# JorisAR/GDPathTracing

Measured on AMD Instinct MI355X. Metric: Mrays/sec at 1920x1080, 8 spp, 4 bounces, higher is better.
Workload: dtype f32

## Files before the change

### gdpathtracing_amd/csrc/jpt_kernels_wf2.hip

```cpp
#include <algorithm>
#include <cstdlib>

#include "jpt_trace_core.h"
#include "jpt_tie_walk.h"
#include "jpt_tuning.h"
#include "jpt_variance.h"

#ifndef JPT_PRIMARY_WAVES
#define JPT_PRIMARY_WAVES 7
#endif

namespace jpt {

namespace {

constexpr int kBlock = kTraceBlock;
constexpr uint32_t kSegments = 256u * JPT_WAVES_PER_SIMD;
struct WfTune {
    int refill_idle;
    int primary_refill_idle;
    int node_min_lanes;
    int leaf_min_lanes;
    int inst_min_lanes;
    int phase_frac16;
    int tail_rounds;
    int tail_lanes;
};

template <bool COUNT, bool W4>
__device__ __forceinline__ bool walk_round(Traversal<COUNT, W4>& tr, bool active, const WideSceneDev& sc,
                                           const typename Traversal<COUNT, W4>::Stack& st, DevCounters& cnt, const WfTune& tune, uint32_t& steps)
{
    const int kNodeMinLanes = tune.node_min_lanes;
    const bool lane0 = (threadIdx.x & 63) == 0;
    if (COUNT && lane0) cnt.phase[0]++;
    const int na = __popcll(__ballot(active));
    const int cap = (na * tune.phase_frac16) >> 4;
    const int lmin = tune.leaf_min_lanes < cap ? tune.leaf_min_lanes : cap;
    const int imin = tune.inst_min_lanes < cap ? tune.inst_min_lanes : cap;
    for (int it = 0; it < 64; it++) {
        if (active && !tr.have && tr.sp > 0) tr.pop_next(st);
        const bool want = active && tr.wants_node();
        const unsigned long long m = __ballot(want);
        if (m == 0 || (it > 0 && __popcll(m) < kNodeMinLanes)) break;
        if (COUNT && lane0) {
            cnt.phase[1]++;
            cnt.phase[2] += (unsigned long long)__popcll(m);
        }
        if (want) tr.node_step(sc, st, cnt);
        if (COUNT && want) steps++;
    }
    bool wl = active && tr.wants_leaf();
    bool wi = active && tr.wants_instance();
    if (W4 && (tune.leaf_min_lanes > 1 || tune.inst_min_lanes > 1)) {
        const int nl = __popcll(__ballot(wl)), ni = __popcll(__ballot(wi));
        const bool nodes_left = __any(active && tr.wants_node()) || __any(active && !tr.have && tr.sp > 0);
        const bool run_l = nl >= lmin || !(nodes_left || ni >= imin);
        const bool run_i = ni >= imin || !(nodes_left || (run_l && nl > 0));
        wl = wl && run_l;
        wi = wi && run_i;
    }
    if (COUNT) {
        const int nl = __popcll(__ballot(wl)), ni = __popcll(__ballot(wi));
        if (lane0 && nl) {
            cnt.phase[3]++;
            cnt.phase[4] += (unsigned long long)nl;
        }
        if (lane0 && ni) {
            cnt.phase[5]++;
            cnt.phase[6] += (unsigned long long)ni;
        }
    }
    if (wl) tr.leaf_step(sc, cnt);
    if (wi) tr.instance_step(sc, st, cnt);
    if (COUNT && (wl || wi)) steps++;
    return active && tr.finished();
}

__device__ __forceinline__ bool in_mask(const unsigned long long m) { return __builtin_amdgcn_inverse_ballot_w64(m); }

struct WalkMasks {
    unsigned long long have = 0ull, in_blas = 0ull;
};
template <bool COUNT, bool W4>
__device__ __forceinline__ unsigned long long walk_round_masked(Traversal<COUNT, W4>& tr, typename Traversal<COUNT, W4>::Masked& ml, WalkMasks& wm,
                                                                const unsigned long long act, const WideSceneDev& sc,
                                                                const typename Traversal<COUNT, W4>::Stack& st, DevCounters& cnt, const WfTune& tune,
                                                                uint32_t& steps)
{
    using Walk = Traversal<COUNT, W4>;
    const int kNodeMinLanes = tune.node_min_lanes;
    const bool lane0 = (threadIdx.x & 63) == 0;
    if (COUNT && lane0) cnt.phase[0]++;
    const int na = __popcll(act);
    const int cap = (na * tune.phase_frac16) >> 4;
    const int lmin = tune.leaf_min_lanes < cap ? tune.leaf_min_lanes : cap;
    const int imin = tune.inst_min_lanes < cap ? tune.inst_min_lanes : cap;
    const uint32_t base = Walk::lds_base(st);
    unsigned long long have_m = wm.have, blas_m = wm.in_blas;
    for (int it = 0; it < 64; it++) {
        const unsigned long long pm = act & ~have_m & __ballot(ml.top > base);
        if (pm) {
            if (in_mask(pm)) tr.cur = tr.pop_at(st, ml.top);
            const unsigned long long sent = pm & __ballot(tr.cur == kSentinel);
            have_m |= pm & ~sent;
            if (sent) {
                blas_m &= ~sent;
                const unsigned long long more = sent & __ballot(ml.top > base);
                if (in_mask(more)) {
                    tr.cur = tr.pop_at(st, ml.top);
                    if (!Walk::kLean || tr.cur >= 0) tr.restore_world();
                }
                have_m |= more;
            }
        }
        const unsigned long long m = act & have_m & __ballot(tr.cur >= 0);
        if (m == 0 || (it > 0 && __popcll(m) < kNodeMinLanes)) break;
        if (COUNT && lane0) {
            cnt.phase[1]++;
            cnt.phase[2] += (unsigned long long)__popcll(m);
        }
        const bool want = in_mask(m);
        ml.in_blas = in_mask(blas_m);
        if (want) tr.template node_step<true>(sc, st, cnt, &ml);
        if (COUNT && want) steps++;
        have_m = (have_m & ~m) | (m & __ballot(ml.k0 < Walk::kNoChild));
    }
    const unsigned long long lf = __ballot(tr.cur < 0), sm = __ballot(ml.top > base);
    const unsigned long long hv = act & have_m;
    unsigned long long wlm = hv & lf & blas_m, wim = hv & lf & ~blas_m;
    if (W4 && (tune.leaf_min_lanes > 1 || tune.inst_min_lanes > 1)) {
        const int nl = __popcll(wlm), ni = __popcll(wim);
        const bool nodes_left = ((hv & ~lf) | (act & ~have_m & sm)) != 0ull;
        const bool run_l = nl >= lmin || !(nodes_left || ni >= imin);
        const bool run_i = ni >= imin || !(nodes_left || (run_l && nl > 0));
        wlm = run_l ? wlm : 0ull;
        wim = run_i ? wim : 0ull;
    }
    if (COUNT) {
        const int nl = __popcll(wlm), ni = __popcll(wim);
        if (lane0 && nl) {
            cnt.phase[3]++;
            cnt.phase[4] += (unsigned long long)nl;
        }
        if (lane0 && ni) {
            cnt.phase[5]++;
            cnt.phase[6] += (unsigned long long)ni;
        }
    }
    const bool wl = in_mask(wlm), wi = in_mask(wim);
    if (wl) tr.leaf_step(sc, cnt);
    if (wi) tr.template instance_step<true>(sc, st, cnt, &ml);
    if (COUNT && (wl || wi)) steps++;
    have_m = (have_m & ~wlm) | wim;
    blas_m |= wim;
    wm.have = have_m;
    wm.in_blas = blas_m;
    return act & ~have_m & ~sm;
}

typedef float jpt_v4f __attribute__((ext_vector_type(4)));
typedef uint32_t jpt_v4u __attribute__((ext_vector_type(4)));
__device__ __forceinline__ float4 stream_ld4(const float4* p)
{
    const jpt_v4f v = __builtin_nontemporal_load(reinterpret_cast<const jpt_v4f*>(p));
    return make_float4(v.x, v.y, v.z, v.w);
}
__device__ __forceinline__ void stream_st4(float4* p, const float4 v)
{
    jpt_v4f w;
    w.x = v.x; w.y = v.y; w.z = v.z; w.w = v.w;
    __builtin_nontemporal_store(w, reinterpret_cast<jpt_v4f*>(p));
}
__device__ __forceinline__ uint4 stream_ldu4(const uint4* p)
{
    const jpt_v4u v = __builtin_nontemporal_load(reinterpret_cast<const jpt_v4u*>(p));
    return make_uint4(v.x, v.y, v.z, v.w);
}
__device__ __forceinline__ void stream_stf(float* p, const float v) { __builtin_nontemporal_store(v, p); }
__device__ __forceinline__ uint32_t stream_ldu(const uint32_t* p) { return __builtin_nontemporal_load(p); }
__device__ __forceinline__ void stream_stu(uint32_t* p, const uint32_t v) { __builtin_nontemporal_store(v, p); }

constexpr uint32_t kHasRadiance = 0x80000000u;
constexpr uint32_t kPathMask = 0x7fffffffu;

struct Wf2Buffers {
    float4* ray_o[2];
    float4* ray_d[2];
    float4* hit_a;
    uint32_t* hit_b;
    float4* thr_q[2];
    float4* thr;
    float4* rad;
    uint32_t* fin8;
    float* first_depth;
    uint32_t* qcount;
    uint32_t* redo_count;
    float4* redo_rec;
    uint32_t redo_cap;
};

struct FastDiv {
    uint32_t d, m;
};
inline FastDiv make_fastdiv(uint32_t d) { return FastDiv{d ? d : 1u, d > 1u ? (uint32_t)(0x100000000ull / d) : 0xffffffffu}; }
__device__ __forceinline__ uint32_t fdiv(uint32_t n, const FastDiv& f)
{
    uint32_t q = __umulhi(n, f.m);
    const uint32_t r = n - q * f.d;
    return r >= f.d ? q + 1u : q;
}

struct Wf2Dims {
    int32_t tile_x0, tile_y0;
    int32_t tiles_x, tiles_y;
    int32_t full_tiles_x, full_tiles_y;
    uint32_t tiles_per_frame;
    uint32_t slots_per_frame;
    uint32_t n_chunks;
    uint32_t seg_cap;
    uint32_t run_shift;
    FastDiv by_tiles_x, by_full_tiles_x;
    FastDiv by_frames;
    int32_t acc_groups = 1;
};

__device__ __forceinline__ void slot_to_pixel(uint32_t slot, const Wf2Dims& dm, int& px, int& ly)
{
    const uint32_t tile = slot >> 6, lane = slot & 63u;
    const uint32_t ty = fdiv(tile, dm.by_tiles_x), tx = tile - ty * (uint32_t)dm.tiles_x;
    const uint32_t ix = lane & 7u, iy = lane >> 3;
    px = (int)((tx + (uint32_t)dm.tile_x0) * 8u + ix);
    ly = (int)((ty + (uint32_t)dm.tile_y0) * 8u + iy);
}

__device__ __forceinline__ void path_slot_frame(uint32_t path, const Wf2Dims& dm, uint32_t n_frames, uint32_t& slot, uint32_t& f)
{
    slot = fdiv(path, dm.by_frames);
    f = path - slot * n_frames;
}

__device__ __forceinline__ void store_final(const Wf2Buffers& wb, int accum_mode, uint32_t p, f3 r)
{
    if (accum_mode == 0) stream_stu(&wb.fin8[p], unorm8(r.x) | (unorm8(r.y) << 8) | (unorm8(r.z) << 16));
    else stream_st4(&wb.rad[p], make_float4(r.x, r.y, r.z, 0.0f));
}

__device__ __forceinline__ bool sky_culled(const SkyCull& cull, int px, int py)
{
    bool outside = cull.n >= 0;
    for (int k = 0; k < 4; k++)
        if (k < cull.n && px >= cull.x0[k] && px <= cull.x1[k] && py >= cull.y0[k] && py <= cull.y1[k]) outside = false;
    return outside;
}

__device__ __forceinline__ uint32_t lanes_below(unsigned long long mask, int lane)
{
    return (uint32_t)__popcll(mask & ((1ull << lane) - 1ull));
}

constexpr int kCoopPool = 64;

__device__ __forceinline__ float wave_min_f(float v)
{
    for (int off = 32; off > 0; off >>= 1) v = fmin_(v, __shfl_xor(v, off));
    return v;
}

template <bool COUNT>
__device__ __forceinline__ TraceHit coop_walk(const WideSceneDev& sc, const typename Traversal<COUNT, true>::Stack st, int32_t* __restrict__ pool,
                                           f3 ro, f3 rd, DevCounters& cnt, const uint32_t pool_stride = 64u)
{
    using Walk = Traversal<COUNT, true>;
    const int lane = threadIdx.x & 63;
    auto pw = [&](uint32_t w) -> int32_t& { return pool[(w >> 6) * pool_stride + (w & 63u)]; };
    constexpr uint32_t kNone = 0xffffffffu;
    Walk tr;
    tr.begin(sc, ro, rd);
    tr.hit.tri = kNone;
    bool active = lane == 0 && tr.have;
    if (lane != 0) tr.have = false;
    uint32_t n_pool = 0;
    uint32_t my_steps = 0;
    for (;;) {
        {
            const unsigned long long idle = __ballot(!active);
            const uint32_t n_idle = (uint32_t)__popcll(idle);
            const uint32_t take = n_pool < n_idle ? n_pool : n_idle;
            if (take) {
                const uint32_t r = lanes_below(idle, lane);
                if (!active && r < take) {
                    const int32_t ref = pw(2u * (n_pool - 1u - r));
                    const uint32_t ctx = (uint32_t)pw(2u * (n_pool - 1u - r) + 1u);
                    tr.sp = 0;
                    tr.cur = ref;
                    tr.have = true;
                    tr.in_blas = (ctx & 1u) != 0u;
                    tr.cur_inst = ctx >> 1;
                    if (tr.in_blas) {
                        const WideInstance* ip = sc.instances + tr.cur_inst;
                        const float4 m0 = ld4(&ip->inv[0]), m1 = ld4(&ip->inv[4]), m2 = ld4(&ip->inv[8]);
                        tr.o = mk3(m0.x * ro.x + m0.w * ro.y + m1.z * ro.z + m2.y, m0.y * ro.x + m1.x * ro.y + m1.w * ro.z + m2.z,
                                   m0.z * ro.x + m1.y * ro.y + m2.x * ro.z + m2.w);
                        tr.d = mk3(m0.x * rd.x + m0.w * rd.y + m1.z * rd.z, m0.y * rd.x + m1.x * rd.y + m1.w * rd.z,
                                   m0.z * rd.x + m1.y * rd.y + m2.x * rd.z);
                    } else {
                        tr.o = ro;
                        tr.d = rd;
                    }
                    tr.set_level();
                    active = true;
                }
                n_pool -= take;
            }
        }
        if (!__any(active)) break;
        if (COUNT && active && (tr.have || tr.sp > 0)) my_steps++;
        if (active && !tr.step(sc, st, cnt)) active = false;
        {
            const float t = wave_min_f(tr.hit.t);
            if (t < tr.hit.t) {
                tr.hit.t = t;
                tr.hit.tri = kNone;
                tr.hit.inst = 0u;
            }
        }
        {
            const uint32_t n_idle = (uint32_t)__popcll(__ballot(!active));
            const uint32_t want = n_idle > n_pool ? n_idle - n_pool : 0u;
            if (want) {
                int32_t top = kSentinel;
                const bool may = active && tr.sp > 0;
                if (may) {
                    const int row = tr.sp - 1;
                    top = row < st.lds_entries ? st.lds[row * st.stride] : (row < st.lds_entries + st.spill_entries ? st.spill[row - st.lds_entries] : kSentinel);
                }
                const bool give = may && top != kSentinel;
                const unsigned long long gm = __ballot(give);
                const uint32_t r = lanes_below(gm, lane);
                const uint32_t room = (uint32_t)kCoopPool - n_pool;
                const uint32_t lim = want < room ? want : room;
                if (give && r < lim) {
                    tr.sp--;
                    pw(2u * (n_pool + r)) = top;
                    pw(2u * (n_pool + r) + 1u) = (int32_t)((tr.in_blas ? 1u : 0u) | (tr.cur_inst << 1));
                }
                const uint32_t given = (uint32_t)__popcll(gm);
                n_pool += given < lim ? given : lim;
            }
        }
        __builtin_amdgcn_fence(__ATOMIC_RELEASE, "wavefront");
        __builtin_amdgcn_wave_barrier();
    }
    if (COUNT) {
        for (int off = 32; off > 0; off >>= 1) my_steps += (uint32_t)__shfl_xor((int)my_steps, off);
        if (lane == 0) count_walk(cnt, my_steps);
    }
    const float best = wave_min_f(tr.hit.t);
    const unsigned long long win = __ballot(tr.hit.tri != kNone && tr.hit.t == best);
    TraceHit out;
    out.t = 1e9f;
    out.u = out.v = 0.0f;
    out.tri = out.inst = 0u;
    out.front = false;
    if (win && best < 1e9f) {
        unsigned long long pick = win;
        if (__popcll(win) > 1) {
            const bool mine = ((win >> lane) & 1ull) != 0ull;
            uint32_t kt = mine ? tr.hit.tri : 0u;
            for (int off = 32; off > 0; off >>= 1) {
                const uint32_t o = (uint32_t)__shfl_xor((int)kt, off);
                kt = o > kt ? o : kt;
            }
            const bool top = mine && tr.hit.tri == kt;
            uint32_t ki = top ? ((tr.hit.inst >> kInstBits) & kInstMask) : 0u;
            for (int off = 32; off > 0; off >>= 1) {
                const uint32_t o = (uint32_t)__shfl_xor((int)ki, off);
                ki = o > ki ? o : ki;
            }
            pick = __ballot(top && ((tr.hit.inst >> kInstBits) & kInstMask) == ki);
        }
        const int w = __ffsll((long long)pick) - 1;
        out.t = best;
        out.u = __shfl(tr.hit.u, w);
        out.v = __shfl(tr.hit.v, w);
        out.tri = (uint32_t)__shfl((int)tr.hit.tri, w);
        out.front = __shfl((int)tr.hit.front, w) != 0;
        const uint32_t wi = (uint32_t)__shfl((int)tr.hit.inst, w);
        const uint32_t found_in = (wi >> kInstBits) & kInstMask;
        const bool tied = __popcll(win) > 1 || (wi & kHitTied) != 0u;
        out.inst = found_in | (found_in << kInstBits) | (tied ? kHitTied : 0u);
    }
    return out;
}

template <bool COUNT>
__device__ __attribute__((noinline)) void coop_walk_call(const WideSceneDev* __restrict__ scp, int32_t* lds_col, int32_t* pool, float ox, float oy,
                                                         float oz, float dx, float dy, float dz, DevCounters* cntp, TraceHit* out)
{
    int32_t spill[kStackSpill + 2];
    const typename Traversal<COUNT, true>::Stack st{lds_col, spill, kTraceBlock, kStackLds - 2, kStackSpill + 2};
    const WideSceneDev sc = *scp;
    DevCounters none = {};
    *out = coop_walk<COUNT>(sc, st, pool, mk3(ox, oy, oz), mk3(dx, dy, dz), COUNT ? *cntp : none, (uint32_t)kTraceBlock);
}


#ifndef JPT_MAX_CHAIN
#define JPT_MAX_CHAIN 4
#endif
constexpr int kMaxChain = JPT_MAX_CHAIN;
template <bool COUNT, bool W4, bool TAIL>
__device__ __forceinline__ void trace_queue(const WideSceneDev& sc, const Wf2Buffers& wb, const Wf2Dims& dm, const int bounce, const WfTune& tune,
                                            const uint32_t seg0, const uint32_t (&end)[kMaxChain], const uint32_t n, int32_t* __restrict__ stack,
                                            uint32_t* __restrict__ s_cursor, DevCounters& cnt)
{
    const int lane = threadIdx.x & 63;
    int32_t spill[kStackSpill];
    const typename Traversal<COUNT, W4>::Stack my_stack{&stack[threadIdx.x], spill, kTraceBlock, kStackLds};
    uint32_t dry_rounds = 0;
    const float4* __restrict__ qo = wb.ray_o[bounce & 1];
    const float4* __restrict__ qd = wb.ray_d[bounce & 1];
    Traversal<COUNT, W4> tr;
    tr.cur = 0;
    WalkMasks wm;
    typename Traversal<COUNT, W4>::Masked ml;
    ml.top = Traversal<COUNT, W4>::lds_base(my_stack);
    ml.k0 = 0u;
    ml.in_blas = false;
    unsigned long long act = 0ull, unsaved = 0ull;
    bool exhausted = false;
    size_t my_loc = 0;
    uint32_t walk_steps = 0;
    auto save_hit = [&]() {
        stream_st4(&wb.hit_a[my_loc], make_float4(tr.hit.t, tr.hit.u, tr.hit.v, __uint_as_float(tr.hit.tri)));
        stream_stu(&wb.hit_b[my_loc], tr.hit.inst | (tr.hit.front ? 0x80000000u : 0u));
    };

    for (;;) {
        const unsigned long long idle = ~act;
        const int n_idle = __popcll(idle);
        if (!exhausted && n_idle >= tune.refill_idle) {
            if (in_mask(unsaved)) save_hit();
            unsaved = 0ull;
            uint32_t start = 0;
            if (lane == 0) start = atomicAdd(s_cursor, (uint32_t)n_idle);
            start = (uint32_t)__builtin_amdgcn_readfirstlane((int)start);
            if (start + (uint32_t)n_idle >= n) exhausted = true;
            if (start < n) {
                const uint32_t idx = start + lanes_below(idle, lane);
                const unsigned long long fill = idle & __ballot(idx < n);
                if (in_mask(fill)) {
                    uint32_t k = 0, first = 0;
                    for (int j = 0; j < kMaxChain - 1; j++)
                        if (idx >= end[j]) {
                            k = (uint32_t)j + 1u;
                            first = end[j];
                        }
                    const size_t loc = (size_t)(seg0 + k) * dm.seg_cap + (idx - first);
                    const float4 ro = stream_ld4(&qo[loc]), rd = stream_ld4(&qd[loc]);
                    tr.begin(sc, mk3(ro.x, ro.y, ro.z), mk3(rd.x, rd.y, rd.z));
                    ml.top = Traversal<COUNT, W4>::lds_base(my_stack);
                    my_loc = loc;
                    walk_steps = 0;
                }
                act |= fill;
                wm.have = sc.n_instances != 0 ? (wm.have | fill) : (wm.have & ~fill);
                wm.in_blas &= ~fill;
            }
        }
        if (act == 0ull) {
            if (exhausted) break;
            continue;
        }
        {
            const unsigned long long done = walk_round_masked<COUNT, W4>(tr, ml, wm, act, sc, my_stack, cnt, tune, walk_steps);
            act &= ~done;
            unsaved |= done;
            if (COUNT) {
                if (in_mask(done)) count_walk(cnt, walk_steps);
            }
            if constexpr (TAIL && W4) {
                if (exhausted && ++dry_rounds >= (uint32_t)tune.tail_rounds && __popcll(act) <= tune.tail_lanes) break;
            }
        }
    }
    if constexpr (TAIL && W4) {
        unsigned long long left = act;
        if (left) {
            if (in_mask(unsaved)) save_hit();
            unsaved = 0ull;
            const int wave_col = (int)(threadIdx.x & ~63u);
            while (left) {
                const int src = __ffsll((long long)left) - 1;
                left &= left - 1ull;
                TraceHit h;
                const WideSceneDev sc_tail = sc;
                coop_walk_call<COUNT>(&sc_tail, &stack[threadIdx.x], &stack[(kStackLds - 2) * kTraceBlock + wave_col], __shfl(tr.wo.x, src),
                                      __shfl(tr.wo.y, src), __shfl(tr.wo.z, src), __shfl(tr.wd.x, src), __shfl(tr.wd.y, src), __shfl(tr.wd.z, src),
                                      COUNT ? &cnt : nullptr, &h);
                if (lane == src) {
                    tr.hit = h;
                    save_hit();
                }
            }
        }
    }
    if (in_mask(unsaved)) save_hit();
}

template <bool COUNT, bool W4, bool TAIL = false>
__global__ __launch_bounds__(kBlock, JPT_WAVES_PER_SIMD) void wf2_trace(WideSceneDev sc, Wf2Buffers wb, Wf2Dims dm, int bounce, WfTune tune,
                                                    int chain, DevCounters* __restrict__ counters)
{
    __shared__ int32_t stack[kStackLds * kBlock];
    __shared__ uint32_t s_cursor;
    const uint32_t seg0 = blockIdx.x * (uint32_t)chain;
    uint32_t end[kMaxChain];
    uint32_t n = 0;
    for (int k = 0; k < kMaxChain; k++) {
        if (k < chain && seg0 + (uint32_t)k < kSegments) n += wb.qcount[(size_t)bounce * kSegments + seg0 + (uint32_t)k];
        end[k] = n;
    }
    if (n == 0) return;
    if (threadIdx.x == 0) s_cursor = 0;
    __syncthreads();
    DevCounters cnt = {};
    trace_queue<COUNT, W4, TAIL>(sc, wb, dm, bounce, tune, seg0, end, n, stack, &s_cursor, cnt);
    if (COUNT) flush_counters(cnt, counters);
}

constexpr float kCellMargin = 0.01f;
__device__ __forceinline__ bool sky_cells_at(const RefCamera& cam, float two_over_w, float two_over_h, float fx, float fy, float w_ref, float& w_out,
                                             float v[3], f3& d)
{
    d = raster_direction_approx(cam, two_over_w, two_over_h, fx, fy, w_out);
    const f3 c = mk3(0.0f, 0.0f, 0.0f) + mk3(1.0f, 1.0f, 1.0f) * sample_sky(d);
    v[0] = clamp_(c.x, 0.0f, 1.0f) * 255.0f + 0.5f;
    v[1] = clamp_(c.y, 0.0f, 1.0f) * 255.0f + 0.5f;
    v[2] = clamp_(c.z, 0.0f, 1.0f) * 255.0f + 0.5f;
    return (w_out * w_ref > 0.0f) && (d.y == d.y);
}
__device__ __forceinline__ float sky_interior_excess(const f3 c[4])
{
    float chord2 = 0.0f, ay = 0.0f;
    for (int i = 0; i < 4; i++) {
        ay = fmax_(ay, __builtin_fabsf(c[i].y));
        for (int j = i + 1; j < 4; j++) {
            const f3 e = c[i] - c[j];
            chord2 = fmax_(chord2, e.x * e.x + e.y * e.y + e.z * e.z);
        }
    }
    if (!(chord2 < 0.2f)) return 1e30f;
    const float theta2 = 1.1f * chord2;
    const float m = fmin_(1.0f, ay + __builtin_sqrtf(theta2));
    return 6.4f * 0.25f * theta2 * m;
}

__global__ __launch_bounds__(kBlock) void wf2_sky_tiles(Wf2Dims dm, FrameParams fp, RefCamera cam, uint32_t* __restrict__ tile_cell)
{
    const uint32_t t = blockIdx.x * kBlock + threadIdx.x;
    if (t >= (uint32_t)dm.full_tiles_x * (uint32_t)dm.full_tiles_y) return;
    const uint32_t fty = fdiv(t, dm.by_full_tiles_x), ftx = t - fty * (uint32_t)dm.full_tiles_x;
    const int tx0 = (int)ftx * 8, ty0 = local_to_global_row((int)fty * 8, fp);
    const float two_over_w = 2.0f / (float)fp.width, two_over_h = 2.0f / (float)fp.height;
    float lo[3] = {1e30f, 1e30f, 1e30f}, hi[3] = {-1e30f, -1e30f, -1e30f};
    f3 cd[4];
    float w0 = 1.0f;
    bool ok = true;
    for (int corner = 0; corner < 4; corner++) {
        float ww, v[3];
        (void)sky_cells_at(cam, two_over_w, two_over_h, (float)(tx0 + 8 * (corner & 1)), (float)(ty0 + 8 * (corner >> 1)), 1.0f, ww, v, cd[corner]);
        if (corner == 0) w0 = ww;
        ok = ok && (ww == ww) && (v[0] == v[0]) && (ww * w0 > 0.0f);
        for (int k = 0; k < 3; k++) {
            lo[k] = fmin_(lo[k], v[k]);
            hi[k] = fmax_(hi[k], v[k]);
        }
    }
    const float excess = sky_interior_excess(cd);
    uint32_t cell = 0x80000000u;
    for (int k = 0; k < 3; k++) {
        const float l = lo[k] - excess, h = hi[k] + excess;
        const float c = __builtin_floorf(l);
        ok = ok && (l - c >= kCellMargin) && (h - c <= 1.0f - kCellMargin) && (h - l < 0.5f);
        cell |= ((uint32_t)c & 255u) << (8 * k);
    }
    tile_cell[t] = ok ? cell : 0u;
}


struct Wf2Nee {
    float4* sh_o;
    float4* sh_d;
    float4* sh_c;
    uint32_t* scount;
    float* pdf;
};
constexpr uint32_t kNeeFinal = 0x80000000u;

__device__ __forceinline__ void nee_land(const Wf2Buffers& wb, int accum_mode, const float4 so, const float4 sc4, bool blocked)
{
    const uint32_t w = __float_as_uint(so.w), p = w & kPathMask;
    const float4 r4 = wb.rad[p];
    f3 r = mk3(r4.x, r4.y, r4.z);
    if (!blocked) r = r + mk3(sc4.x, sc4.y, sc4.z);
    if (w & kNeeFinal) store_final(wb, accum_mode, p, r);
    else if (!blocked) wb.rad[p] = make_float4(r.x, r.y, r.z, 0.0f);
}

constexpr int kOccBlock = 64;
template <bool COUNT, bool W4>
__global__ __launch_bounds__(kOccBlock) void wf2_occlude(WideSceneDev sc, Wf2Buffers wb, Wf2Dims dm, FrameParams fp, int bounce, Wf2Nee nee,
                                                         DevCounters* __restrict__ counters)
{
    constexpr int kDepth = kStackLds + kStackSpill;
    __shared__ int32_t stack[kDepth * kOccBlock];
    const uint32_t seg = blockIdx.y;
    const uint32_t i = blockIdx.x * kOccBlock + threadIdx.x;
    if (i >= nee.scount[(size_t)bounce * kSegments + seg]) return;
    const size_t at = (size_t)seg * dm.seg_cap + i;
    const float4 so = stream_ld4(&nee.sh_o[at]), sd = stream_ld4(&nee.sh_d[at]), sc4 = stream_ld4(&nee.sh_c[at]);
    const typename Traversal<COUNT, W4>::Stack st{&stack[threadIdx.x], nullptr, kOccBlock, kDepth, 0};
    DevCounters cnt = {};
    Traversal<COUNT, W4> tr;
    tr.begin(sc, mk3(so.x, so.y, so.z), mk3(sd.x, sd.y, sd.z));
    while (tr.hit.t >= 1e9f && tr.step(sc, st, cnt)) {
    }
    nee_land(wb, fp.accum_mode, so, sc4, tr.hit.t < 1e9f);
    if (COUNT) flush_counters(cnt, counters);
}

template <bool COUNT, bool W4>
__global__ __launch_bounds__(kOccBlock) void wf2_occlude_lt(WideSceneDev sc, Wf2Buffers wb, Wf2Dims dm, FrameParams fp, int bounce, Wf2Nee nee,
                                                            DevCounters* __restrict__ counters)
{
    constexpr int kDepth = kStackLds + kStackSpill;
    __shared__ int32_t stack[kDepth * kOccBlock];
    const uint32_t seg = blockIdx.y;
    const uint32_t i = blockIdx.x * kOccBlock + threadIdx.x;
    if (i >= nee.scount[(size_t)bounce * kSegments + seg]) return;
    const size_t at = (size_t)seg * dm.seg_cap + i;
    const float4 so = stream_ld4(&nee.sh_o[at]), sd = stream_ld4(&nee.sh_d[at]), sc4 = stream_ld4(&nee.sh_c[at]);
    const typename Traversal<COUNT, W4>::Stack st{&stack[threadIdx.x], nullptr, kOccBlock, kDepth, 0};
    DevCounters cnt = {};
    Traversal<COUNT, W4> tr;
    tr.begin(sc, mk3(so.x, so.y, so.z), mk3(sd.x, sd.y, sd.z));
    const float tmax = sd.w;
    tr.hit.t = tmax;
    while (tr.hit.t >= tmax && tr.step(sc, st, cnt)) {
    }
    nee_land(wb, fp.accum_mode, so, sc4, tr.hit.t < tmax);
    if (COUNT) flush_counters(cnt, counters);
}

#define JPT_ENV 0
#include "jpt_wf2_paths.h"
#undef JPT_ENV
#define JPT_ENV 1
#include "jpt_wf2_paths.h"
#undef JPT_ENV
#define JPT_ENV 2
#include "jpt_wf2_paths.h"
#undef JPT_ENV
#define JPT_ENV 3
#include "jpt_wf2_paths.h"
#undef JPT_ENV
#define JPT_ENV 4
#include "jpt_wf2_paths.h"
#undef JPT_ENV
#define JPT_LENS 1
#define JPT_ENV 0
#include "jpt_wf2_paths.h"
#undef JPT_ENV
#define JPT_ENV 1
#include "jpt_wf2_paths.h"
#undef JPT_ENV
#undef JPT_LENS
#define JPT_CAMERA_MODEL 1
#define JPT_ENV 0
#include "jpt_wf2_paths.h"
#undef JPT_ENV
#define JPT_ENV 1
#include "jpt_wf2_paths.h"
#undef JPT_ENV
#undef JPT_CAMERA_MODEL
#define JPT_BAKE 1
#define JPT_ENV 0
#include "jpt_wf2_paths.h"
#undef JPT_ENV
#define JPT_ENV 1
#include "jpt_wf2_paths.h"
#undef JPT_ENV
#undef JPT_BAKE
#define JPT_PROBE 1
#define JPT_ENV 0
#include "jpt_wf2_paths.h"
#undef JPT_ENV
#define JPT_ENV 1
#include "jpt_wf2_paths.h"
#undef JPT_ENV
#undef JPT_PROBE
#define JPT_CUBE 1
#define JPT_ENV 0
#include "jpt_wf2_paths.h"
#undef JPT_ENV
#define JPT_ENV 1
#include "jpt_wf2_paths.h"
#undef JPT_ENV
#undef JPT_CUBE

struct TileWindow {
    int x0, y0, nx, ny;
};
TileWindow full_window(int width, int local_rows) { return TileWindow{0, 0, (width + 7) / 8, (local_rows + 7) / 8}; }

TileWindow cull_window(const SkyCull& cull, const FrameParams& fp)
{
    const TileWindow full = full_window(fp.width, fp.local_rows);
    if (cull.n < 0) return full;
    const TileWindow none{0, 0, 1, 1};
    int gx0 = INT32_MAX, gy0 = INT32_MAX, gx1 = INT32_MIN, gy1 = INT32_MIN;
    for (int k = 0; k < 4 && k < cull.n; k++) {
        if (cull.x0[k] > cull.x1[k] || cull.y0[k] > cull.y1[k]) continue;
        gx0 = std::min(gx0, cull.x0[k]);
        gy0 = std::min(gy0, cull.y0[k]);
        gx1 = std::max(gx1, cull.x1[k]);
        gy1 = std::max(gy1, cull.y1[k]);
    }
    gx0 = std::max(gx0, 0);
    gy0 = std::max(gy0, 0);
    gx1 = std::min(gx1, fp.width - 1);
    gy1 = std::min(gy1, fp.height - 1);
    if (gx0 > gx1 || gy0 > gy1) return none;
    const int world = fp.world > 0 ? fp.world : 1;
    const int ty0 = gy0 / 8 - fp.rank, ty1 = gy1 / 8 - fp.rank;
    if (ty1 < 0) return none;
    const int lt0 = ty0 <= 0 ? 0 : (ty0 + world - 1) / world, lt1 = std::min(ty1 / world, full.ny - 1);
    if (lt0 > lt1) return none;
    return TileWindow{gx0 / 8, lt0, gx1 / 8 - gx0 / 8 + 1, lt1 - lt0 + 1};
}

Wf2Dims make_dims(int width, int local_rows, int n_frames, const TileWindow& win)
{
    Wf2Dims dm;
    dm.tile_x0 = win.x0;
    dm.tile_y0 = win.y0;
    dm.tiles_x = win.nx;
    dm.tiles_y = win.ny;
    dm.full_tiles_x = (width + 7) / 8;
    dm.full_tiles_y = (local_rows + 7) / 8;
    dm.by_full_tiles_x = make_fastdiv((uint32_t)dm.full_tiles_x);
    dm.tiles_per_frame = (uint32_t)dm.tiles_x * (uint32_t)dm.tiles_y;
    dm.slots_per_frame = dm.tiles_per_frame * 64u;
    dm.n_chunks = dm.tiles_per_frame * (uint32_t)n_frames;
    const uint32_t per_segment = dm.n_chunks / kSegments;
    const uint32_t run_shift = per_segment >= 512u ? 2u : (per_segment >= 256u ? 1u : 0u);
    dm.run_shift = run_shift;
    const uint32_t n_runs = (dm.n_chunks + (1u << run_shift) - 1u) >> run_shift;
    dm.seg_cap = (((n_runs + kSegments - 1u) / kSegments) << run_shift) * 64u;
    dm.by_tiles_x = make_fastdiv((uint32_t)dm.tiles_x);
    dm.by_frames = make_fastdiv((uint32_t)(n_frames > 0 ? n_frames : 1));
    return dm;
}

}

size_t wf2_sky_tile_count(int width, int local_rows) { return (size_t)((width + 7) / 8) * (size_t)((local_rows + 7) / 8); }
void launch_sky_tiles(hipStream_t stream, const FrameParams& fp, const RefCamera& cam, uint32_t* tile_cell)
{
    const Wf2Dims dm = make_dims(fp.width, fp.local_rows, 1, full_window(fp.width, fp.local_rows));
    const uint32_t n_tiles = (uint32_t)dm.full_tiles_x * (uint32_t)dm.full_tiles_y;
    if (n_tiles) hipLaunchKernelGGL(wf2_sky_tiles, dim3((n_tiles + kBlock - 1) / kBlock), dim3(kBlock), 0, stream, dm, fp, cam, tile_cell);
}
uint32_t wf2_segments() { return kSegments; }
uint32_t trace_stack_capacity() { return (uint32_t)(kStackLds + kStackSpill); }

static void group_frames(int n_frames, int groups, int g, int& first, int& count)
{
// ... 315 lines not shown
```

### gdpathtracing_amd/csrc/jpt_trace_core.h

```cpp
#pragma once

#include "jpt_kernels.h"
#include "jpt_shade.h"

namespace jpt {

constexpr int kTraceBlock = 256;
#ifndef JPT_STACK_LDS
#define JPT_STACK_LDS 20
#endif
#ifndef JPT_WAVES_PER_SIMD
#define JPT_WAVES_PER_SIMD 7
#endif
constexpr int kStackLds = JPT_STACK_LDS;
constexpr int kStackSpill = 76;
constexpr int32_t kSentinel = 0x7fffffff;

struct WideSceneDev {
    const WideNode* __restrict__ blas_nodes;
    const WideNode* __restrict__ tlas_nodes;
    const WideNodeQ* __restrict__ nodesq;
    const WideTri* __restrict__ tris;
    const WideInstance* __restrict__ instances;
    int32_t tlas_root;
// ... 29 lines not shown
struct Traversal {
    static constexpr bool kLean = W4;
    f3 wo, wd, wrD;
    f3 o, d, rD;
    f3 ood;
    f3 xrD;
    TraceHit hit;
    int32_t cur;
    int sp;
    uint32_t cur_inst;
    bool in_blas, have;

    struct Stack {
        int32_t* __restrict__ lds;
        int32_t* __restrict__ spill;
        int stride = kTraceBlock;
        int lds_entries = kStackLds;
        int spill_entries = kStackSpill;
    };

    __device__ __forceinline__ void push(const Stack& st, int32_t v)
    {
        if (sp < st.lds_entries) st.lds[sp * st.stride] = v;
        else if (sp < st.lds_entries + st.spill_entries) st.spill[sp - st.lds_entries] = v;
        sp++;
    }
    __device__ __forceinline__ int32_t pop(const Stack& st)
    {
        sp--;
        if (st.lds_entries <= 0) return sp < st.spill_entries ? st.spill[sp] : kSentinel;
        const int row = sp < st.lds_entries ? sp : st.lds_entries - 1;
        int32_t v = st.lds[row * st.stride];
        if (__builtin_expect(sp >= st.lds_entries, 0)) v = sp < st.lds_entries + st.spill_entries ? st.spill[sp - st.lds_entries] : kSentinel;
        return v;
    }

    typedef __attribute__((address_space(3))) int32_t LdsWord;
    struct Masked {
        uint32_t top;
        uint32_t k0;
        bool in_blas;
    };
    static constexpr uint32_t kNoChild = 0x7f800000u;
    static __device__ __forceinline__ uint32_t lds_base(const Stack& st) { return (uint32_t)(uintptr_t)(LdsWord*)st.lds; }
    static __device__ __forceinline__ uint32_t lds_limit(const Stack& st) { return lds_base(st) + (uint32_t)(st.lds_entries * st.stride) * 4u; }
    static __device__ __forceinline__ LdsWord* lds_at(uint32_t a) { return (LdsWord*)(uintptr_t)a; }
    __device__ __forceinline__ void push_at(const Stack& st, uint32_t& top, int32_t v) const
    {
        const uint32_t lim = lds_limit(st);
        if (__builtin_expect(top < lim, 1)) *lds_at(top) = v;
        else {
            const int k = (int)((top - lim) / ((uint32_t)st.stride * 4u));
            if (k < st.spill_entries) st.spill[k] = v;
        }
        top += (uint32_t)st.stride * 4u;
    }
    __device__ __forceinline__ int32_t pop_at(const Stack& st, uint32_t& top) const
    {
        const uint32_t lim = lds_limit(st), last = lim - (uint32_t)st.stride * 4u;
        top -= (uint32_t)st.stride * 4u;
        int32_t v = *lds_at(top < last ? top : last);
        if (__builtin_expect(top >= lim, 0)) {
            const int k = (int)((top - lim) / ((uint32_t)st.stride * 4u));
            v = k < st.spill_entries ? st.spill[k] : kSentinel;
        }
        return v;
    }
    __device__ __forceinline__ void restore_world()
    {
        o = wo;
        d = wd;
        if (kLean) asm volatile("" : "+v"(d.x), "+v"(d.y), "+v"(d.z));
        if (kLean) set_level();
        else rD = wrD;
    }

    __device__ __forceinline__ void begin(const WideSceneDev& sc, f3 ro, f3 rd)
    {
        wo = ro;
        wd = rd;
        o = ro;
        d = rd;
        set_level();
        wrD = (kLean && REACH) ? xrD : rD;
        hit.t = 1e9f;
        hit.u = hit.v = 0.0f;
        hit.tri = hit.inst = 0;
        hit.front = false;
        sp = 0;
        in_blas = false;
        cur_inst = 0;
        cur = sc.tlas_root;
        have = sc.n_instances != 0;
    }

    __device__ __forceinline__ void set_level()
    {
        if (kLean) {
            rD = mk3(__builtin_amdgcn_fmed3f(__builtin_amdgcn_rcpf(d.x), -kRcpClamp, kRcpClamp), __builtin_amdgcn_fmed3f(__builtin_amdgcn_rcpf(d.y), -kRcpClamp, kRcpClamp),
                     __builtin_amdgcn_fmed3f(__builtin_amdgcn_rcpf(d.z), -kRcpClamp, kRcpClamp));
            ood = mk3(-(o.x * rD.x), -(o.y * rD.y), -(o.z * rD.z));
            if (REACH) xrD = rcp3(d);
        } else {
            rD = rcp3(d);
        }
    }


    __device__ __forceinline__ bool wants_node() const { return have && cur >= 0; }
    __device__ __forceinline__ bool wants_leaf() const { return have && cur < 0 && in_blas; }
    __device__ __forceinline__ bool wants_instance() const { return have && cur < 0 && !in_blas; }
    __device__ __forceinline__ bool finished() const { return !have && sp == 0; }

    template <bool MASKED = false>
    __device__ __forceinline__ void node_step4(const WideSceneDev& sc, const Stack& st, DevCounters& cnt, Masked* ms = nullptr)
    {
        const char* __restrict__ base = reinterpret_cast<const char*>(sc.nodesq);
        const uint32_t rec = (uint32_t)cur << 6;
        const float4 h0 = ld4(base + rec);
        const float4 h1 = ld4(base + (rec + 16u));
        const float4 h2 = ld4(base + (rec + 32u));
        const float4 cf = ld4(base + (rec + 48u));
        node_step4_rec<MASKED>(h0, h1, h2, cf, st, cnt, ms);
    }
    template <bool MASKED = false>
    __device__ __forceinline__ void node_step4_rec(const float4 h0, const float4 h1, const float4 h2, const float4 cf, const Stack& st, DevCounters& cnt,
                                                   Masked* ms = nullptr)
    {
        static_assert(!(MASKED && REACH), "the masked rounds do not walk with reach records");
        if (COUNT) {
            if (MASKED ? ms->in_blas : in_blas) cnt.blas_expand++;
            else cnt.tlas_expand++;
        }
        const float ax = h0.w * rD.x, ay = h1.x * rD.y, az = h1.y * rD.z;
        const float bx = __builtin_fmaf(h0.x, rD.x, ood.x), by = __builtin_fmaf(h0.y, rD.y, ood.y), bz = __builtin_fmaf(h0.z, rD.z, ood.z);
        const float mx = __builtin_fmaf(kWalkSlackOverEps, __builtin_fabsf(ax), __builtin_fabsf(bx)) + __builtin_fabsf(ood.x);
        const float my = __builtin_fmaf(kWalkSlackOverEps, __builtin_fabsf(ay), __builtin_fabsf(by)) + __builtin_fabsf(ood.y);
        const float mz = __builtin_fmaf(kWalkSlackOverEps, __builtin_fabsf(az), __builtin_fabsf(bz)) + __builtin_fabsf(ood.z);
        const float nbx = __builtin_fmaf(-kWalkEps, mx, bx), fbx = __builtin_fmaf(kWalkEps, mx, bx);
        const float nby = __builtin_fmaf(-kWalkEps, my, by), fby = __builtin_fmaf(kWalkEps, my, by);
        const float nbz = __builtin_fmaf(-kWalkEps, mz, bz), fbz = __builtin_fmaf(kWalkEps, mz, bz);
        const bool negx = __float_as_int(d.x) < 0, negy = __float_as_int(d.y) < 0, negz = __float_as_int(d.z) < 0;
        const uint32_t lox = __float_as_uint(h1.z), loy = __float_as_uint(h1.w), loz = __float_as_uint(h2.x);
        const uint32_t hix = __float_as_uint(h2.y), hiy = __float_as_uint(h2.z), hiz = __float_as_uint(h2.w);
        const uint32_t nwx = negx ? hix : lox, fwx = negx ? lox : hix;
        const uint32_t nwy = negy ? hiy : loy, fwy = negy ? loy : hiy;
        const uint32_t nwz = negz ? hiz : loz, fwz = negz ? loz : hiz;
        int32_t r0 = __float_as_int(cf.x), r1 = __float_as_int(cf.y), r2 = __float_as_int(cf.z), r3 = __float_as_int(cf.w);
        constexpr uint32_t kInvalid = 0x7f800000u;
        const float tcur = hit.t;
        auto key = [&](int k, int32_t ch) -> uint32_t {
            const float qnx = (float)((nwx >> (8 * k)) & 255u), qny = (float)((nwy >> (8 * k)) & 255u), qnz = (float)((nwz >> (8 * k)) & 255u);
            const float qfx = (float)((fwx >> (8 * k)) & 255u), qfy = (float)((fwy >> (8 * k)) & 255u), qfz = (float)((fwz >> (8 * k)) & 255u);
            const float t_in = fmax_(fmax_(fmax_(__builtin_fmaf(qnx, ax, nbx), __builtin_fmaf(qny, ay, nby)), __builtin_fmaf(qnz, az, nbz)), 0.0f);
            const float t_out = fmin_(fmin_(fmin_(__builtin_fmaf(qfx, ax, fbx), __builtin_fmaf(qfy, ay, fby)), __builtin_fmaf(qfz, az, fbz)), tcur);
            return ((t_in <= t_out) & (ch != kEmptyChild)) ? __float_as_uint(t_in) : kInvalid;
        };
        uint32_t k0 = key(0, r0), k1 = key(1, r1), k2 = key(2, r2), k3 = key(3, r3);
        auto cswap = [](uint32_t& ka, uint32_t& kb, int32_t& ra, int32_t& rb) {
            const bool lt = ka < kb;
            const uint32_t klo = lt ? ka : kb, khi = lt ? kb : ka;
            const int32_t rlo = lt ? ra : rb, rhi = lt ? rb : ra;
            ka = klo; kb = khi; ra = rlo; rb = rhi;
        };
        cswap(k0, k1, r0, r1);
        cswap(k2, k3, r2, r3);
        cswap(k0, k2, r0, r2);
        cswap(k1, k3, r1, r3);
        cswap(k1, k2, r1, r2);
        if constexpr (MASKED) {
            ms->k0 = k0;
            cur = k0 < kInvalid ? r0 : cur;
            if (k1 < kInvalid) {
                if (k2 < kInvalid) {
                    if (k3 < kInvalid) push_at(st, ms->top, r3);
                    push_at(st, ms->top, r2);
                }
                push_at(st, ms->top, r1);
            }
        } else {
            have = k0 < kInvalid;
            cur = have ? r0 : cur;
            if (k1 < kInvalid) {
                if (k2 < kInvalid) {
                    if (k3 < kInvalid) push(st, r3);
                    push(st, r2);
                }
                push(st, r1);
            }
        }
    }

    template <bool MASKED = false>
    __device__ __forceinline__ void node_step(const WideSceneDev& sc, const Stack& st, DevCounters& cnt, Masked* ms = nullptr)
    {
        if (W4) {
            node_step4<MASKED>(sc, st, cnt, ms);
            return;
        }
        const bool in_blas = MASKED ? ms->in_blas : this->in_blas;
        const WideNode* n = (in_blas ? sc.blas_nodes : sc.tlas_nodes) + cur;
        const float4 a = ld4(&n->lmin[0]);
        const float4 b = ld4(&n->lmax[1]);
        const float4 c = ld4(&n->rmin[2]);
        const float4 e = ld4(&n->left);
        if (COUNT) {
            if (in_blas) cnt.blas_expand++;
            else cnt.tlas_expand++;
        }
        const float d1 = slab(o, rD, a.x, a.y, a.z, a.w, b.x, b.y);
        const float d2 = slab(o, rD, b.z, b.w, c.x, c.y, c.z, c.w);
        const int32_t left = __float_as_int(e.x), right = __float_as_int(e.y);
        const bool lv = d1 < hit.t, rv = d2 < hit.t;
        const bool left_first = d1 < d2;
        const int32_t near_ref = left_first ? left : right, far_ref = left_first ? right : left;
        const bool near_v = left_first ? lv : rv, far_v = left_first ? rv : lv;
        if constexpr (MASKED) {
            if (near_v) {
                if (far_v) push_at(st, ms->top, far_ref);
                cur = near_ref;
            } else if (far_v) {
                cur = far_ref;
            }
            ms->k0 = (near_v || far_v) ? 0u : kNoChild;
        } else {
            have = false;
            if (near_v) {
                if (far_v) push(st, far_ref);
                cur = near_ref;
                have = true;
            } else if (far_v) {
                cur = far_ref;
                have = true;
            }
        }
    }

    __device__ __forceinline__ void leaf_step(const WideSceneDev& sc, DevCounters& cnt)
    {
        const uint32_t bits = (uint32_t)~cur;
        const uint32_t first = bits & kLeafFirstMask;
        const uint32_t count = (bits >> kLeafCountShift) + 1u;
        have = false;
        for (uint32_t i = 0; i < count; i++) {
            const uint32_t ti = first + i;
            const WideTri* tp = sc.tris + ti;
            const float4 q0 = ld4(&tp->v0[0]);
            const float4 q1 = ld4(&tp->e1[0]);
            const float4 q2 = ld4(&tp->e2[0]);
            if (COUNT) cnt.tri_tests++;
            const f3 v0 = mk3(q0.x, q0.y, q0.z), edge1 = mk3(q1.x, q1.y, q1.z), edge2 = mk3(q2.x, q2.y, q2.z);
            if (W4) {
                const f3 pvec = cross3(d, edge2);
                const float det = dot3(edge1, pvec);
                const float invDet = 1.0f / det;
                const f3 tvec = o - v0;
                const float u = dot3(tvec, pvec) * invDet;
                const f3 qvec = cross3(tvec, edge1);
                const float v = dot3(d, qvec) * invDet;
                const float t = dot3(edge2, qvec) * invDet;
                bool out = (__builtin_fabsf(det) < 1e-5f) | (u < 0.0f) | (u > 1.0f) | (v < 0.0f) | (u + v > 1.0f) |
                           (t < 0.0f) | (t > hit.t);
                if (REACH) {
                    if (!out && !reaches_triangle(sc, ti)) out = true;
                }
                float facing = dot3(mk3(q0.w, q1.w, q2.w), d);
                asm volatile("" : "+v"(facing));
                const bool front = facing > 0.0f;
                if (!out) {
                    const bool closer = t < hit.t;
                    hit.inst = ((closer ? cur_inst : hit.inst) & kInstMask) | (cur_inst << kInstBits) | (closer ? 0u : kHitTied);
                    hit.t = t;
                    hit.u = u;
                    hit.v = v;
                    hit.tri = ti;
                    hit.front = front;
                }
            } else {
                const f3 pvec = cross3(d, edge2);
                const float det = dot3(edge1, pvec);
                if (__builtin_fabsf(det) < 1e-5f) continue;
                const float invDet = 1.0f / det;
                const f3 tvec = o - v0;
                const float u = dot3(tvec, pvec) * invDet;
                if (u < 0.0f || u > 1.0f) continue;
                const f3 qvec = cross3(tvec, edge1);
                const float v = dot3(d, qvec) * invDet;
                if (v < 0.0f || u + v > 1.0f) continue;
                const float t = dot3(edge2, qvec) * invDet;
                if (t < 0.0f || t > hit.t) continue;
                if (REACH) {
                    if (!reaches_triangle(sc, ti)) continue;
                }
                hit.inst = (((t < hit.t) ? cur_inst : hit.inst) & kInstMask) | (cur_inst << kInstBits);
                hit.t = t;
                hit.u = u;
                hit.v = v;
                hit.tri = ti;
                hit.front = dot3(cross3(edge1, edge2), d) > 0.0f;
            }
        }
    }

    __device__ __forceinline__ bool reaches_triangle(const WideSceneDev& sc, uint32_t ti) const
    {
        const float4 a = ld4(&sc.reach_tri[ti].lo[0]), b = ld4(&sc.reach_tri[ti].hi[0]);
        if (__float_as_uint(a.w) != 0u) return true;
        return slab(o, kLean ? xrD : rD, a.x, a.y, a.z, b.x, b.y, b.z) < 1e30f;
    }

    template <bool MASKED = false>
    __device__ __forceinline__ void instance_step(const WideSceneDev& sc, const Stack& st, DevCounters& cnt, Masked* ms = nullptr)
    {
        static_assert(!(MASKED && REACH), "the masked rounds do not walk with reach records");
        cur_inst = (uint32_t)~cur;
        if (REACH) {
            if (sc.n_instances > 1u) {
                const float4 a = ld4(&sc.reach_inst[cur_inst].lo[0]), b = ld4(&sc.reach_inst[cur_inst].hi[0]);
                if (!(slab(wo, wrD, a.x, a.y, a.z, b.x, b.y, b.z) < 1e30f)) {
                    if (kLean) {
                        o = wo;
                        d = wd;
                        set_level();
                    }
                    have = false;
                    return;
                }
            }
        }
        const WideInstance* ip = sc.instances + cur_inst;
        const float4 m0 = ld4(&ip->inv[0]);
        const float4 m1 = ld4(&ip->inv[4]);
        const float4 m2 = ld4(&ip->inv[8]);
        const int32_t root = ip->root;
        if (COUNT) cnt.inst_visits++;
        o = mk3(m0.x * wo.x + m0.w * wo.y + m1.z * wo.z + m2.y, m0.y * wo.x + m1.x * wo.y + m1.w * wo.z + m2.z,
                m0.z * wo.x + m1.y * wo.y + m2.x * wo.z + m2.w);
        d = mk3(m0.x * wd.x + m0.w * wd.y + m1.z * wd.z, m0.y * wd.x + m1.x * wd.y + m1.w * wd.z,
                m0.z * wd.x + m1.y * wd.y + m2.x * wd.z);
        set_level();
        if constexpr (MASKED) {
            push_at(st, ms->top, kSentinel);
            cur = root;
        } else {
            in_blas = true;
            push(st, kSentinel);
            cur = root;
            have = true;
        }
    }

    template <bool ON_DEMAND = false>
    __device__ __forceinline__ void pop_next(const Stack& st)
    {
        cur = pop(st);
        if (cur == kSentinel) {
            in_blas = false;
            if (sp == 0) return;
            cur = pop(st);
            if (!kLean || cur >= 0) {
                o = wo;
                d = wd;
                if (kLean && ON_DEMAND) asm volatile("" : "+v"(d.x), "+v"(d.y), "+v"(d.z));
                if (kLean) set_level();
                else rD = wrD;
            }
        }
        have = true;
    }

    __device__ __forceinline__ bool step(const WideSceneDev& sc, const Stack& st, DevCounters& cnt)
    {
        if (!have) {
            if (sp == 0) return false;
            pop_next(st);
            if (!have) return false;
        }
        if (cur >= 0) node_step(sc, st, cnt);
        else if (in_blas) leaf_step(sc, cnt);
        else instance_step(sc, st, cnt);
        return true;
    }
};

}
```

Before: 29520.

## Split two-triangle leaves across idle lanes in masked leaf rounds

When few lanes take a leaf step and every leaf holds at most two triangles, each taking lane borrows an idle lane through ds_permute/bpermute. The borrowed lane tests the second triangle and sends t/u/v and a verdict back, so both triangles are tested in one pass instead of a serial loop. This is meant to cut leaf-phase latency and divergence in half-empty waves, at the cost of many cross-lane permutes and a separate triangle-test path. It only applies in the non-tail W4 walk.

```diff
diff --git a/gdpathtracing_amd/csrc/jpt_kernels_wf2.hip b/gdpathtracing_amd/csrc/jpt_kernels_wf2.hip
--- a/gdpathtracing_amd/csrc/jpt_kernels_wf2.hip
+++ b/gdpathtracing_amd/csrc/jpt_kernels_wf2.hip
@@ -82,7 +82,7 @@
 struct WalkMasks {
     unsigned long long have = 0ull, in_blas = 0ull;
 };
-template <bool COUNT, bool W4>
+template <bool COUNT, bool W4, bool PAIR = false>
 __device__ __forceinline__ unsigned long long walk_round_masked(Traversal<COUNT, W4>& tr, typename Traversal<COUNT, W4>::Masked& ml, WalkMasks& wm,
                                                                 const unsigned long long act, const WideSceneDev& sc,
                                                                 const typename Traversal<COUNT, W4>::Stack& st, DevCounters& cnt, const WfTune& tune,
@@ -149,7 +149,14 @@
         }
     }
     const bool wl = in_mask(wlm), wi = in_mask(wim);
-    if (wl) tr.leaf_step(sc, cnt);
+    if constexpr (PAIR && W4) {
+        const unsigned long long big = wlm & __ballot((uint32_t)tr.cur <= ~(2u << kLeafCountShift));
+        const bool pairs = wlm != 0ull && __popcll(wlm) <= 32 && big == 0ull;
+        if (pairs) tr.leaf_pair_step(sc, cnt, wlm, threadIdx.x & 63u);
+        if (in_mask(pairs ? 0ull : wlm)) tr.leaf_step(sc, cnt);
+    } else {
+        if (wl) tr.leaf_step(sc, cnt);
+    }
     if (wi) tr.template instance_step<true>(sc, st, cnt, &ml);
     if (COUNT && (wl || wi)) steps++;
     have_m = (have_m & ~wlm) | wim;
@@ -474,7 +481,7 @@
             continue;
         }
         {
-            const unsigned long long done = walk_round_masked<COUNT, W4>(tr, ml, wm, act, sc, my_stack, cnt, tune, walk_steps);
+            const unsigned long long done = walk_round_masked<COUNT, W4, W4 && !TAIL>(tr, ml, wm, act, sc, my_stack, cnt, tune, walk_steps);
             act &= ~done;
             unsaved |= done;
             if (COUNT) {
diff --git a/gdpathtracing_amd/csrc/jpt_trace_core.h b/gdpathtracing_amd/csrc/jpt_trace_core.h
--- a/gdpathtracing_amd/csrc/jpt_trace_core.h
+++ b/gdpathtracing_amd/csrc/jpt_trace_core.h
@@ -355,6 +355,74 @@
         }
     }
 
+    __device__ __forceinline__ void leaf_pair_step(const WideSceneDev& sc, DevCounters& cnt, const unsigned long long takers, const uint32_t lane)
+    {
+        static_assert(W4 && !REACH, "the paired leaf phase is the native tree's, in the tracing launches");
+        const bool taker = __builtin_amdgcn_inverse_ballot_w64(takers);
+        const uint32_t n_takers = (uint32_t)__popcll(takers);
+        const uint32_t below = __builtin_amdgcn_mbcnt_hi((uint32_t)(takers >> 32), __builtin_amdgcn_mbcnt_lo((uint32_t)takers, 0u));
+        const uint32_t lane4 = lane << 2;
+        const uint32_t by_rank = (uint32_t)__builtin_amdgcn_ds_permute((int)(taker ? below << 2 : 63u * 4u), (int)lane4);
+        const uint32_t hrank = lane - below;
+        const uint32_t lender = (uint32_t)__builtin_amdgcn_ds_bpermute((int)(hrank << 2), (int)by_rank);
+        const uint32_t src4 = taker ? lane4 : lender;
+        const uint32_t bits = (uint32_t)__builtin_amdgcn_ds_bpermute((int)src4, ~cur);
+        const unsigned long long helpers = ~takers & __ballot(hrank < n_takers) & __ballot(bits >= (1u << kLeafCountShift));
+        if (__builtin_amdgcn_inverse_ballot_w64(takers | helpers)) {
+            const f3 po = mk3(__int_as_float(__builtin_amdgcn_ds_bpermute((int)src4, __float_as_int(o.x))),
+                              __int_as_float(__builtin_amdgcn_ds_bpermute((int)src4, __float_as_int(o.y))),
+                              __int_as_float(__builtin_amdgcn_ds_bpermute((int)src4, __float_as_int(o.z))));
+            const f3 pd = mk3(__int_as_float(__builtin_amdgcn_ds_bpermute((int)src4, __float_as_int(d.x))),
+                              __int_as_float(__builtin_amdgcn_ds_bpermute((int)src4, __float_as_int(d.y))),
+                              __int_as_float(__builtin_amdgcn_ds_bpermute((int)src4, __float_as_int(d.z))));
+            const uint32_t ti = (bits & kLeafFirstMask) + (taker ? 0u : 1u);
+            const WideTri* tp = sc.tris + ti;
+            const float4 q0 = ld4(&tp->v0[0]);
+            const float4 q1 = ld4(&tp->e1[0]);
+            const float4 q2 = ld4(&tp->e2[0]);
+            if (COUNT) cnt.tri_tests++;
+            const f3 v0 = mk3(q0.x, q0.y, q0.z), edge1 = mk3(q1.x, q1.y, q1.z), edge2 = mk3(q2.x, q2.y, q2.z);
+            const f3 pvec = cross3(pd, edge2);
+            const float det = dot3(edge1, pvec);
+            const float invDet = 1.0f / det;
+            const f3 tvec = po - v0;
+            const float u = dot3(tvec, pvec) * invDet;
+            const f3 qvec = cross3(tvec, edge1);
+            const float v = dot3(pd, qvec) * invDet;
+            const float t = dot3(edge2, qvec) * invDet;
+            const bool out = (__builtin_fabsf(det) < 1e-5f) | (u < 0.0f) | (u > 1.0f) | (v < 0.0f) | (u + v > 1.0f) | (t < 0.0f);
+            const float facing = dot3(mk3(q0.w, q1.w, q2.w), pd);
+            const bool front = facing > 0.0f;
+            const uint32_t verdict = out ? 0u : (front ? 2u : 1u);
+            const uint32_t dump4 = (uint32_t)(__ffsll((long long)~takers) - 1) << 2;
+            const uint32_t dst4 = taker ? dump4 : src4;
+            const float t1 = __int_as_float(__builtin_amdgcn_ds_permute((int)dst4, __float_as_int(t)));
+            const float u1 = __int_as_float(__builtin_amdgcn_ds_permute((int)dst4, __float_as_int(u)));
+            const float v1 = __int_as_float(__builtin_amdgcn_ds_permute((int)dst4, __float_as_int(v)));
+            const uint32_t verdict1 = (uint32_t)__builtin_amdgcn_ds_permute((int)dst4, (int)verdict);
+            if (taker) {
+                if (!(out | (t > hit.t))) {
+                    const bool closer = t < hit.t;
+                    hit.inst = ((closer ? cur_inst : hit.inst) & kInstMask) | (cur_inst << kInstBits) | (closer ? 0u : kHitTied);
+                    hit.t = t;
+                    hit.u = u;
+                    hit.v = v;
+                    hit.tri = ti;
+                    hit.front = front;
+                }
+                if (!((bits < (1u << kLeafCountShift)) | (verdict1 == 0u) | (t1 > hit.t))) {
+                    const bool closer = t1 < hit.t;
+                    hit.inst = ((closer ? cur_inst : hit.inst) & kInstMask) | (cur_inst << kInstBits) | (closer ? 0u : kHitTied);
+                    hit.t = t1;
+                    hit.u = u1;
+                    hit.v = v1;
+                    hit.tri = ti + 1u;
+                    hit.front = verdict1 == 2u;
+                }
+            }
+        }
+    }
+
     __device__ __forceinline__ bool reaches_triangle(const WideSceneDev& sc, uint32_t ti) const
     {
         const float4 a = ld4(&sc.reach_tri[ti].lo[0]), b = ld4(&sc.reach_tri[ti].hi[0]);
```

After: 29940, median of 6. 1.01x the previous value.
